# EavnJeong/IEF-VAD

Measured on AMD Instinct MI355X. Metric: snippets/sec at [B,T=256,d=768], higher is better.
Workload: dtype f32 emulated: exact 3-term bf16 split of both fp32 operands, 6 bf16 MFMA products, fp32 accumulate

## Files before the change

### ief-vad_amd/csrc/gemm_bf16.h

```cpp
#pragma once
#include "common.h"
#include "gemm_f32.h"

typedef __bf16 bf16_t;
typedef __bf16 bf16x8 __attribute__((ext_vector_type(8)));
typedef __bf16 bf16x4 __attribute__((ext_vector_type(4)));

struct GemmBProblem {
    const bf16_t* A;
    const bf16_t* W;
    const float* bias;
    float* C;
    bf16_t* Cb;
    const float* R;
    float* C2;
    const float* amaxA;
    const float* amaxW;
    float* amaxC;
};

struct GemmBArgs {
    GemmBProblem p[2];
    int M, N, K;
    int lda, ldc;
// ... 130 lines not shown
#pragma unroll
    for (int a = 0; a < 2; ++a) {
#pragma unroll
        for (int b = 0; b < 2; ++b)
#pragma unroll
            for (int r = 0; r < 16; ++r)
                E[((r & 3) + 8 * (r >> 2) + 4 * h) * GEMMB_EPI_LD + b * 32 + i] = acc[a][b][r];
#pragma unroll
        for (int u = 0; u < 8; ++u) {
            const int lr = rq + 4 * u;
            f32x4 v = *(const f32x4*)(E + lr * GEMMB_EPI_LD + 4 * cq);
            v = v + bv;
            if (epi == EPI_QKV) v = v * scale;
            else if (epi == EPI_BIAS_RELU) {
#pragma unroll
                for (int e = 0; e < 4; ++e) v[e] = (v[e] < 0.f) ? 0.f : v[e];
            } else if (epi == EPI_BIAS_RESID) v = v + res[a * 8 + u];
            else if (epi == EPI_REFINE) v = res[a * 8 + u] - alpha * v;
            const size_t o = (size_t)(mrow + a * 32 + 4 * u) * ldc + nn;
            if (Cb32) *(f32x4*)(Cb32 + o) = v;
            if (Cb16) {
                bf16x4 w;
#pragma unroll
                for (int e = 0; e < 4; ++e) w[e] = (bf16_t)v[e];
                *(bf16x4*)(Cb16 + o) = w;
            }
        }
    }
}


#define GB2_BARRIER()                       \
    do {                                    \
        asm volatile("" ::: "memory");      \
        __builtin_amdgcn_s_barrier();       \
        asm volatile("" ::: "memory");      \
    } while (0)
#define GB2_BM 128
#define GB2_BN 256
#define GB2_BK 32
#define GB2_SLOT ((GB2_BM + GB2_BN) * 16)
#define GB2_STAGES 3
#define GB2_EPI_LD 132
#define GB2_LDS_BYTES (GB2_STAGES * GB2_SLOT * 4)

#ifndef GB2_NT_STORES
#define GB2_NT_STORES 1
#endif
#if GB2_NT_STORES
#define GB2_STORE(ptr, val) __builtin_nontemporal_store((val), (ptr))
#else
#define GB2_STORE(ptr, val) (*(ptr) = (val))
#endif
template <bool MF16, int PASSES>
__device__ __forceinline__ void gemm_wave_epilogue(const GemmBArgs& args, const GemmBProblem& P, float* smem, int m0, int n0,
                                                   int wrow0, int wcol0, f32x16 (&acc)[PASSES][4],
                                                   f32x4 (&acc16)[2 * PASSES][8], float cscale = 1.0f, float* amax_out = nullptr) {
    const int lane = threadIdx.x & 63, wave = threadIdx.x >> 6;
    const int i = lane & 31, h = lane >> 5;
    const int r16 = lane & 15, q16 = lane >> 4;
    const int epi = args.epi, ldc = args.ldc;
    const float alpha = args.alpha;
    const int rq = lane >> 5, cq = lane & 31;
    const int ncol = n0 + wcol0 + 4 * cq;
    const bool has_resid = (epi == EPI_BIAS_RESID || epi == EPI_REFINE || epi == EPI_GATE);
    float* E = smem + wave * (32 * GB2_EPI_LD);
    const f32x4 bv = *(const f32x4*)(P.bias + ncol);
    float* C32 = P.C;
    bf16_t* C16 = P.Cb;
    int nn = ncol;
    f32x4 scale = {1.f, 1.f, 1.f, 1.f};
    if (epi == EPI_HEADS && ncol >= ldc) { C32 = P.C2; nn = ncol - ldc; }
    if (epi == EPI_QKV && ncol < args.qcols) scale = f32x4{alpha, alpha, alpha, alpha};
    float vmax = 0.f;
    const bool wide16 = C16 && !C32 && !has_resid && !amax_out && (epi == EPI_BIAS || epi == EPI_QKV || epi == EPI_BIAS_RELU);
    if (wide16) {
        const int rq4 = lane >> 4, c8 = lane & 15;
        const int ncol8 = n0 + wcol0 + 8 * c8;
        const f32x4 b0 = *(const f32x4*)(P.bias + ncol8), b1 = *(const f32x4*)(P.bias + ncol8 + 4);
        const float sc = (epi == EPI_QKV && ncol8 < args.qcols) ? alpha : 1.f;
#pragma unroll
        for (int a = 0; a < PASSES; ++a) {
            if constexpr (MF16) {
#pragma unroll
                for (int x = 0; x < 2; ++x)
#pragma unroll
                    for (int b = 0; b < 8; ++b)
#pragma unroll
                        for (int r = 0; r < 4; ++r)
                            E[(x * 16 + 4 * q16 + r) * GB2_EPI_LD + b * 16 + r16] = acc16[2 * a + x][b][r];
            } else {
#pragma unroll
                for (int b = 0; b < 4; ++b)
#pragma unroll
                    for (int r = 0; r < 16; ++r)
                        E[((r & 3) + 8 * (r >> 2) + 4 * h) * GB2_EPI_LD + b * 32 + i] = acc[a][b][r];
            }
#pragma unroll
            for (int u = 0; u < 8; ++u) {
                const int row = rq4 + 4 * u;
                f32x4 v0 = *(const f32x4*)(E + row * GB2_EPI_LD + 8 * c8);
                f32x4 v1 = *(const f32x4*)(E + row * GB2_EPI_LD + 8 * c8 + 4);
                v0 = v0 * cscale + b0;
                v1 = v1 * cscale + b1;
                if (epi == EPI_QKV) { v0 = v0 * sc; v1 = v1 * sc; }
                bf16x8 w;
#pragma unroll
                for (int e = 0; e < 4; ++e) {
                    float x0 = v0[e], x1 = v1[e];
                    if (epi == EPI_BIAS_RELU) { x0 = x0 < 0.f ? 0.f : x0; x1 = x1 < 0.f ? 0.f : x1; }
                    w[e] = (bf16_t)x0;
                    w[4 + e] = (bf16_t)x1;
                }
                GB2_STORE((bf16x8*)(C16 + (size_t)(m0 + wrow0 + a * 32 + row) * ldc + ncol8), w);
            }
        }
        return;
    }
#pragma unroll
    for (int a = 0; a < PASSES; ++a) {
        const int mrow = m0 + wrow0 + a * 32 + rq;
        f32x4 res[16];
        if (has_resid) {
#pragma unroll
            for (int u = 0; u < 16; ++u)
                res[u] = *(const f32x4*)(P.R + (size_t)(mrow + 2 * u) * ldc + ncol);
        }
        if constexpr (MF16) {
#pragma unroll
            for (int x = 0; x < 2; ++x)
#pragma unroll
                for (int b = 0; b < 8; ++b)
#pragma unroll
                    for (int r = 0; r < 4; ++r)
                        E[(x * 16 + 4 * q16 + r) * GB2_EPI_LD + b * 16 + r16] = acc16[2 * a + x][b][r];
        } else {
#pragma unroll
            for (int b = 0; b < 4; ++b)
#pragma unroll
                for (int r = 0; r < 16; ++r)
                    E[((r & 3) + 8 * (r >> 2) + 4 * h) * GB2_EPI_LD + b * 32 + i] = acc[a][b][r];
        }
#pragma unroll
        for (int u = 0; u < 16; ++u) {
            f32x4 v = *(const f32x4*)(E + (rq + 2 * u) * GB2_EPI_LD + 4 * cq);
            v = v * cscale + bv;
            if (epi == EPI_QKV) v = v * scale;
            else if (epi == EPI_BIAS_RELU) {
#pragma unroll
                for (int e = 0; e < 4; ++e) v[e] = (v[e] < 0.f) ? 0.f : v[e];
            } else if (epi == EPI_BIAS_RESID) v = v + res[u];
            else if (epi == EPI_REFINE) v = res[u] - alpha * v;
            else if (epi == EPI_GATE) {
#pragma unroll
                for (int e = 0; e < 4; ++e) v[e] = res[u][e] > 0.f ? alpha * v[e] : 0.f;
            }
            const size_t o = (size_t)(mrow + 2 * u) * ldc + nn;
            if (C32) GB2_STORE((f32x4*)(C32 + o), v);
            if (C16) {
                bf16x4 w;
#pragma unroll
                for (int e = 0; e < 4; ++e) w[e] = (bf16_t)v[e];
                GB2_STORE((bf16x4*)(C16 + o), w);
            }
            if (amax_out) {
#pragma unroll
                for (int e = 0; e < 4; ++e) vmax = amax_fold(vmax, v[e]);
            }
        }
    }
// ... 263 lines not shown
```

### ief-vad_amd/csrc/gemm_f32.h

```cpp
#pragma once
#include "common.h"

enum GemmEpilogue {
    EPI_BIAS = 0,
    EPI_QKV = 1,
    EPI_BIAS_RELU = 2,
    EPI_BIAS_RESID = 3,
    EPI_REFINE = 4,
    EPI_HEADS = 5,
    EPI_GATE = 6,
};

struct GemmProblem {
    const float* A;
    const float* W;
    const float* bias;
    float* C;
    const float* R;
    float* C2;
};

struct GemmArgs {
    GemmProblem p[2];
    int M, N, K;
    int lda, ldc;
    int epi;
    float alpha;
    int qcols;
};

#define GEMM_BM 128
#define GEMM_BN 128
#define GEMM_BK 32


template <int TM, int TN>
__device__ __forceinline__ void gemm_prefetch_residual(const GemmArgs& args, const GemmProblem& P, f32x16 (&res)[TM][TN],
                                                       int m0, int n0, int wr, int wc, int i, int h) {
    const int epi = args.epi, ldc = args.ldc;
    if (epi == EPI_BIAS_RESID || epi == EPI_REFINE) {
#pragma unroll
        for (int b = 0; b < TN; ++b)
#pragma unroll
            for (int a = 0; a < TM; ++a)
#pragma unroll
                for (int r = 0; r < 16; ++r)
                    res[a][b][r] = P.R[(size_t)(m0 + wr * 32 * TM + a * 32 + 4 * h + (r & 3) + 8 * (r >> 2)) * ldc +
                                       n0 + wc * 32 * TN + b * 32 + i];
    }
}

template <int TM, int TN>
__device__ __forceinline__ void gemm_epilogue(const GemmArgs& args, const GemmProblem& P, f32x16 (&acc)[TM][TN],
                                              f32x16 (&res)[TM][TN], int m0, int n0, int wr, int wc, int i, int h) {
    const int epi = args.epi, ldc = args.ldc;
    const float alpha = args.alpha;
#pragma unroll
    for (int b = 0; b < TN; ++b) {
        const int n = n0 + wc * 32 * TN + b * 32 + i;
        const float bv = P.bias[n];
        float* Cb = P.C;
        int nn = n;
        float scale = 1.f;
// ... 350 lines not shown
```

### ief-vad_amd/csrc/gemm_split.h

```cpp
#pragma once
#include "gemm_bf16.h"

#ifndef GS_EXP_NODMA
#define GS_EXP_NODMA 0
#endif
#ifndef GS_EXP_NOSPLIT
#define GS_EXP_NOSPLIT 0
#endif
#ifndef GS_EXP_NOBAR
#define GS_EXP_NOBAR 0
#endif
#ifndef GS_PN
#define GS_PN 6
#endif
#define GS_BM 128
#define GS_BK 32
#define GS_A_SLOT (GS_BM * 32)
#define GS_BN_OF(NA) ((NA) == 4 ? 256 : 128)
#define GS_LDS_BYTES_OF(NA) ((2 * GS_A_SLOT + 2 * 3 * GS_BN_OF(NA) * 16) * 4)
#define GS_BN GS_BN_OF(4)
#define GS_LDS_BYTES GS_LDS_BYTES_OF(4)

typedef float f32x2 __attribute__((ext_vector_type(2)));
typedef __bf16 bf16x2 __attribute__((ext_vector_type(2)));
// ... 290 lines not shown
            mfma_row(B, 0, w[1]);                                                                    \
            mfma_row(B, 0, w[0]);                                                                    \
            if (!GS_EXP_NOSPLIT) {                                                                              \
                if (GS_NSPLIT(B) >= 1) split_half(B, v0);                                                       \
                if (GS_NSPLIT(B) == 2) split_half((B) + 1, v1);                                                 \
            }                                                                                                   \
            if ((B) == 7) {                                                                                     \
                _Pragma("unroll") for (int a = 0; a < NA; ++a)                                                  \
                    _Pragma("unroll") for (int p = 0; p < NP; ++p) ap[a][p] = an[a][p];                         \
            }                                                                                                   \
            _Pragma("unroll") for (int d = 0; d < GS_NDMA(B); ++d) dma(GS_NDMA(B) * (B) + d);                   \
            if (GS_NREAD(B) > 0) __builtin_amdgcn_sched_group_barrier(0x100, GS_NREAD(B) > 0 ? GS_NREAD(B) : 1, 0); \
            GS_SLOT(B, 0) GS_SLOT(B, 1) GS_SLOT(B, 2) GS_SLOT(B, 3) GS_SLOT(B, 4) GS_SLOT(B, 5)                 \
            GS_SLOT(B, 6) GS_SLOT(B, 7) GS_SLOT(B, 8) GS_SLOT(B, 9) GS_SLOT(B, 10) GS_SLOT(B, 11)               \
            GS_SLOT(B, 12) GS_SLOT(B, 13) GS_SLOT(B, 14) GS_SLOT(B, 15) GS_SLOT(B, 16) GS_SLOT(B, 17)           \
            GS_SLOT(B, 18) GS_SLOT(B, 19) GS_SLOT(B, 20) GS_SLOT(B, 21) GS_SLOT(B, 22) GS_SLOT(B, 23)           \
            GS_FENCE();                                                                                         \
            if ((B) < 7) {                                                                                      \
                _Pragma("unroll") for (int p = 0; p < NP; ++p) w[p] = wn[p];                                    \
                if (GS_NAREAD(B) >= 1) v0 = vn0;                                                                \
                if (GS_NAREAD(B) == 2) v1 = vn1;                                                                \
            }                                                                                                   \
        }
        GS_STEP(0) GS_STEP(1) GS_STEP(2) GS_STEP(3) GS_STEP(4) GS_STEP(5) GS_STEP(6) GS_STEP(7)
#undef GS_STEP
#undef GS_SLOT
#undef GS_VSLOT
#undef GS_NVALU
#undef GS_NDMA
#undef GS_NREAD
#undef GS_NAREAD
#undef GS_NSPLIT
        GS_DIAG_STAMP(0)
        asm volatile("s_waitcnt vmcnt(0)" ::: "memory");
        asm volatile("s_waitcnt lgkmcnt(0)" ::: "memory");
        GS_DIAG_STAMP(1)
        if (!GS_EXP_NOBAR) GB2_BARRIER();
        GS_DIAG_STAMP(2)
    }
#ifdef GB2_CLOCK_DIAG
    if (threadIdx.x == 0 && P.C2) {
        unsigned long long* dg = (unsigned long long*)P.C2 + 2 * (blockIdx.x + gridDim.x * blockIdx.z);
        dg[0] = __builtin_amdgcn_s_memtime() - dg_c0;
        dg[1] = __builtin_amdgcn_s_memrealtime() - dg_r0;
        unsigned long long* dx = (unsigned long long*)P.C2 + 2 * gridDim.x * gridDim.z + 3 * (blockIdx.x + gridDim.x * blockIdx.z);
        dx[0] = dg_acc[0]; dx[1] = dg_acc[1]; dx[2] = dg_acc[2];
    }
    const unsigned long long dg_loop_end = __builtin_amdgcn_s_memtime();
#endif
#undef GS_PIPE
#undef GS_FENCE
#undef GLDS16
    f32x16 unused[NA / 2][4];
    gemm_wave_epilogue<true, NA / 2>(args, P, smem, m0, n0, wrow0, wcol0, unused, acc16, cscale, F16 ? P.amaxC : nullptr);
#ifdef GB2_CLOCK_DIAG
    if (threadIdx.x == 0 && P.C2) {
        unsigned long long* dy = (unsigned long long*)P.C2 + 5 * gridDim.x * gridDim.z + 2 * (blockIdx.x + gridDim.x * blockIdx.z);
        dy[0] = dg_c0 - dg_entry;
        dy[1] = __builtin_amdgcn_s_memtime() - dg_loop_end;
    }
#endif
}

__global__ __launch_bounds__(256, 1) void iefvad_gemm_split_kernel(GemmBArgs args) {
    extern __shared__ __attribute__((aligned(16))) float smem[];
    gemm_split_body<4>(args, smem);
}

__global__ __launch_bounds__(256, 2) void iefvad_gemm_split_n128_kernel(GemmBArgs args) {
    extern __shared__ __attribute__((aligned(16))) float smem[];
    gemm_split_body<2>(args, smem);
}

__global__ __launch_bounds__(256, 2) void iefvad_gemm_split_f16_n128_kernel(GemmBArgs args) {
    extern __shared__ __attribute__((aligned(16))) float smem[];
    gemm_split_body<2, true>(args, smem);
}

#ifdef GS_EXPERIMENT_F16
__global__ __launch_bounds__(256, 1) void iefvad_gemm_split_f16_kernel(GemmBArgs args) {
    extern __shared__ __attribute__((aligned(16))) float smem[];
    gemm_split_body<4, true>(args, smem);
}
#endif

__global__ __launch_bounds__(256) void iefvad_split_planes_f16_kernel(const float* __restrict__ src, _Float16* __restrict__ planes,
                                                                      size_t n, const float* __restrict__ amax) {
    const float scale = __builtin_ldexpf(1.0f, 13 - amax_exponent(amax_read(amax)));
    const size_t stride = (size_t)gridDim.x * blockDim.x * 4;
    for (size_t i = ((size_t)blockIdx.x * blockDim.x + threadIdx.x) * 4; i < n; i += stride) {
        Split4 s;
        s.r = *(const f32x4*)(src + i) * scale;
#pragma unroll
        for (int p = 0; p < 2; ++p) {
            unsigned d0, d1;
            s.plane_f16(d0, d1, p < 1);
            *(uint2*)(planes + (size_t)p * n + i) = make_uint2(d0, d1);
        }
    }
}
```

### ief-vad_amd/csrc/iefvad.hip

```cpp
#include "../../include/iefvad.h"

#include <hip/hip_runtime.h>
#include <math.h>
#include <stdarg.h>
#include <stdio.h>
#include <stdlib.h>
#include <string.h>

#include <algorithm>
#include <exception>
#include <new>
#include <thread>
#include <vector>

#include "attention_f32.h"
#include "attention_bf16.h"
#include "attention_pbf16.h"
#include "attention_split.h"
#include "common.h"
#include "gather.h"
#include "gemm_f32.h"
#include "gemm_bf16.h"
#include "gemm_split.h"
#include "rowops.h"
// ... 13 lines not shown
static thread_local char g_err[512] = "";

static int fail(const char* fmt, ...) {
    va_list ap;
    va_start(ap, fmt);
    vsnprintf(g_err, sizeof(g_err), fmt, ap);
    va_end(ap);
    return 1;
}

#define HIP_TRY(expr)                                                                            \
    do {                                                                                         \
        hipError_t e_ = (expr);                                                                  \
        if (e_ != hipSuccess) return fail("%s failed: %s (%s:%d)", #expr, hipGetErrorString(e_), \
                                          __FILE__, __LINE__);                                   \
    } while (0)

struct iefvad_handle {
    iefvad_config cfg;
    int D, DH;
    int device;
    bool weights_set;
    bool no_heads_fusion, no_ln_fusion;
    char* iproj_stream[2][IEFVAD_MAX_LAYERS];
    char* heads_stream;
    int chain_min_blocks;
    int rowblock_min_wgs;
    bool no_inproj_chain;
    char* oproj_stream[2][IEFVAD_MAX_LAYERS];
    bool dense_encoder;
    bool persist;
    bool train_attn_unfused;
    bool hostpipe_trace;
    bool no_chain;
    char* chain_stream;
    float* arena;
    size_t arena_floats;
    float* in_w[2][IEFVAD_MAX_LAYERS];
    float* in_b[2][IEFVAD_MAX_LAYERS];
    float* out_w[2][IEFVAD_MAX_LAYERS];
    float* out_b[2][IEFVAD_MAX_LAYERS];
    float* norm_w[2][IEFVAD_MAX_LAYERS];
    float* norm_b[2][IEFVAD_MAX_LAYERS];
    float* whiten_w[2];
    float* whiten_b[2];
    float* head_w[2];
    float* head_b[2];
    float* ref_w1[IEFVAD_MAX_STEPS];
    float* ref_b1[IEFVAD_MAX_STEPS];
    float* ref_w2[IEFVAD_MAX_STEPS];
    float* ref_b2[IEFVAD_MAX_STEPS];
    float* cls_w;
    float* cls_b;
    bf16_t* arena_b;
    bf16_t* in_wb[2][IEFVAD_MAX_LAYERS];
    bf16_t* out_wb[2][IEFVAD_MAX_LAYERS];
    bf16_t* head_wb[2];
    bf16_t* ref_w1b[IEFVAD_MAX_STEPS];
    bf16_t* ref_w2b[IEFVAD_MAX_STEPS];
    bf16_t* arena_s;
    bf16_t* in_ws[2][IEFVAD_MAX_LAYERS];
    bf16_t* out_ws[2][IEFVAD_MAX_LAYERS];
    bf16_t* head_ws[2];
    bf16_t* ref_w1s[IEFVAD_MAX_STEPS];
    bf16_t* ref_w2s[IEFVAD_MAX_STEPS];
    _Float16* arena_h;
    float* amax_dev;
    _Float16* in_wh[2][IEFVAD_MAX_LAYERS];  const float* in_wa[2][IEFVAD_MAX_LAYERS];
    _Float16* out_wh[2][IEFVAD_MAX_LAYERS]; const float* out_wa[2][IEFVAD_MAX_LAYERS];
    _Float16* head_wh[2];                   const float* head_wa[2];
    _Float16* ref_w1h[IEFVAD_MAX_STEPS];    const float* ref_w1a[IEFVAD_MAX_STEPS];
    _Float16* ref_w2h[IEFVAD_MAX_STEPS];    const float* ref_w2a[IEFVAD_MAX_STEPS];
    struct EventPool* events;
    struct GraphCache* graphs;
    struct MetaRing* meta;
    int num_cus;
    bf16_t* arena_st; float* zero_bias; bool tplanes_valid;
    bf16_t* in_wst[2][IEFVAD_MAX_LAYERS]; bf16_t* out_wst[2][IEFVAD_MAX_LAYERS]; bf16_t* head_wst[2];
    bf16_t* ref_w1st[IEFVAD_MAX_STEPS]; bf16_t* ref_w2st[IEFVAD_MAX_STEPS];
    struct HostPipe* hostpipe;
    struct TrainState* train;
    const float* row_scale[2];
};
static const int kAmaxActBase = 256;
static int amax_act_tensors(int L, int K) { return 2 + 6 * L + 2 * K + 1; }
static size_t amax_words(int L, int K, int mb_chunks) {
    return (size_t)kAmaxActBase * IEF_AMAX_FLOATS + (size_t)amax_act_tensors(L, K) * mb_chunks * IEF_AMAX_PARTS;
}

static const int kDefaultMicroBatchF32 = 256;
static const int kDefaultMicroBatchBF16 = 1024;

static int micro_batch(const iefvad_handle* h) {
    if (h->cfg.micro_batch > 0) return h->cfg.micro_batch < 16384 ? h->cfg.micro_batch : 16384;
    return h->cfg.compute == IEFVAD_COMPUTE_F32 ? kDefaultMicroBatchF32 : kDefaultMicroBatchBF16;
}

extern "C" int iefvad_abi_version(void) { return IEFVAD_ABI_VERSION; }

extern "C" const char* iefvad_last_error(void) { return g_err; }

#define IEF_D512 512

static int create_impl(const char* who, bool allow_512, const iefvad_config* cfg, iefvad_handle** out) {
    if (!cfg || !out) return fail("%s: null argument", who);
    *out = nullptr;
// ... 221 lines not shown
    for (int i = 0; i < count; ++i) {
        if (!src[i] || !planes[i] || rows[i] < 0) return fail("iefvad_split_bf16x3_many: entry %d is null or has negative rows", i);
        if (((uintptr_t)src[i] | (uintptr_t)planes[i]) & 15) return fail("iefvad_split_bf16x3_many: entry %d is not 16-byte aligned", i);
        if (int rc = sm.add(src[i], (bf16_t*)planes[i], n[i], rows[i])) return rc;
    }
    return sm.flush();
}

extern "C" int iefvad_split_bf16x3(const float* src, void* planes, size_t n, void* stream) {
    if (!src || !planes) return fail("iefvad_split_bf16x3: null argument");
    return launch_split_planes(src, (bf16_t*)planes, n, (hipStream_t)stream);
}

#define COPY_MANY_MAX 96
struct CopyManyArgs {
    float* dst[COPY_MANY_MAX];
    const float* src[COPY_MANY_MAX];
    unsigned count[COPY_MANY_MAX];
    int n;
};
__global__ __launch_bounds__(256) void iefvad_copy_many_kernel(CopyManyArgs a) {
    float* d = a.dst[blockIdx.y];
    const float* s = a.src[blockIdx.y];
    const unsigned n = a.count[blockIdx.y];
    const unsigned tid = blockIdx.x * 256 + threadIdx.x, nth = gridDim.x * 256;
    if ((((uintptr_t)d | (uintptr_t)s) & 15) == 0) {
        const unsigned n4 = n >> 2;
        for (unsigned i = tid; i < n4; i += nth) ((f32x4*)d)[i] = ((const f32x4*)s)[i];
        for (unsigned i = (n4 << 2) + tid; i < n; i += nth) d[i] = s[i];
    } else {
        for (unsigned i = tid; i < n; i += nth) d[i] = s[i];
    }
}

extern "C" int iefvad_set_weights(iefvad_handle* h, const iefvad_weights* w, void* stream_) {
    if (!h || !w) return fail("iefvad_set_weights: null argument");
    hipStream_t stream = (hipStream_t)stream_;
    const int L = h->cfg.num_layers, K = h->cfg.num_steps;
    const size_t D = h->D, DD = D * D;
    for (int m = 0; m < 2; ++m) {
        for (int l = 0; l < L; ++l)
            if (!w->in_proj_w[m][l] || !w->in_proj_b[m][l] || !w->out_proj_w[m][l] || !w->out_proj_b[m][l] ||
                !w->norm_w[m][l] || !w->norm_b[m][l])
                return fail("iefvad_set_weights: null encoder weight (modality %d layer %d)", m, l);
        if (!w->whiten_w[m] || !w->whiten_b[m] || !w->mu_w[m] || !w->mu_b[m] || !w->logvar_w[m] || !w->logvar_b[m])
            return fail("iefvad_set_weights: null head weight (modality %d)", m);
    }
    for (int k = 0; k < K; ++k)
        if (!w->ref_w1[k] || !w->ref_b1[k] || !w->ref_w2[k] || !w->ref_b2[k])
            return fail("iefvad_set_weights: null refinement weight (step %d)", k);
    if (!w->cls_w || !w->cls_b) return fail("iefvad_set_weights: null classifier weight");

    const size_t total = 2 * L * (3 * DD + 3 * D + DD + D + 2 * D) + 2 * (2 * D) + 2 * (2 * DD + 2 * D) +
                         (size_t)K * (2 * DD + 2 * D) + D + 4;
    if (!h->arena) {
        HIP_TRY(hipSetDevice(h->device));
        HIP_TRY(hipMalloc((void**)&h->arena, total * sizeof(float)));
        h->arena_floats = total;
    }
    float* p = h->arena;
    CopyManyArgs cm;
    cm.n = 0;
    auto flush = [&]() -> hipError_t {
        if (cm.n == 0) return hipSuccess;
        hipLaunchKernelGGL(iefvad_copy_many_kernel, dim3(32, cm.n), dim3(256), 0, stream, cm);
        cm.n = 0;
        return hipGetLastError();
    };
    auto put = [&](float** dst, const float* src, size_t n) -> hipError_t {
        *dst = p;
        p += n;
        cm.dst[cm.n] = *dst; cm.src[cm.n] = src; cm.count[cm.n] = (unsigned)n;
        if (++cm.n == COPY_MANY_MAX) return flush();
        return hipSuccess;
    };
    for (int m = 0; m < 2; ++m) {
        for (int l = 0; l < L; ++l) {
            HIP_TRY(put(&h->in_w[m][l], w->in_proj_w[m][l], 3 * DD));
            HIP_TRY(put(&h->in_b[m][l], w->in_proj_b[m][l], 3 * D));
            HIP_TRY(put(&h->out_w[m][l], w->out_proj_w[m][l], DD));
            HIP_TRY(put(&h->out_b[m][l], w->out_proj_b[m][l], D));
            HIP_TRY(put(&h->norm_w[m][l], w->norm_w[m][l], D));
            HIP_TRY(put(&h->norm_b[m][l], w->norm_b[m][l], D));
        }
        HIP_TRY(put(&h->whiten_w[m], w->whiten_w[m], D));
        HIP_TRY(put(&h->whiten_b[m], w->whiten_b[m], D));
        HIP_TRY(put(&h->head_w[m], w->mu_w[m], DD));
        float* dummy;
        HIP_TRY(put(&dummy, w->logvar_w[m], DD));
        HIP_TRY(put(&h->head_b[m], w->mu_b[m], D));
        HIP_TRY(put(&dummy, w->logvar_b[m], D));
    }
    for (int k = 0; k < K; ++k) {
        HIP_TRY(put(&h->ref_w1[k], w->ref_w1[k], DD));
        HIP_TRY(put(&h->ref_b1[k], w->ref_b1[k], D));
        HIP_TRY(put(&h->ref_w2[k], w->ref_w2[k], DD));
        HIP_TRY(put(&h->ref_b2[k], w->ref_b2[k], D));
    }
    HIP_TRY(put(&h->cls_w, w->cls_w, D));
    HIP_TRY(put(&h->cls_b, w->cls_b, 1));
    HIP_TRY(flush());
    if ((size_t)(p - h->arena) > h->arena_floats) return fail("iefvad_set_weights: arena overflow");
    if (h->cfg.compute == IEFVAD_COMPUTE_BF16) {
        const size_t nb = 2 * (size_t)L * (3 * DD + DD) + 2 * (2 * DD) + (size_t)K * 2 * DD;
        if (!h->arena_b) HIP_TRY(hipMalloc((void**)&h->arena_b, nb * sizeof(bf16_t)));
        bf16_t* q = h->arena_b;
        auto conv = [&](bf16_t** dst, const float* src, size_t n) -> int {
            *dst = q;
            q += n;
            return launch_cast<float>(src, nullptr, nullptr, nullptr, *dst, nullptr, n, 1, stream);
        };
        for (int m = 0; m < 2; ++m) {
            for (int l = 0; l < L; ++l) {
                if (int rc = conv(&h->in_wb[m][l], h->in_w[m][l], 3 * DD)) return rc;
                if (int rc = conv(&h->out_wb[m][l], h->out_w[m][l], DD)) return rc;
            }
            if (int rc = conv(&h->head_wb[m], h->head_w[m], 2 * DD)) return rc;
        }
        for (int k = 0; k < K; ++k) {
            if (int rc = conv(&h->ref_w1b[k], h->ref_w1[k], DD)) return rc;
            if (int rc = conv(&h->ref_w2b[k], h->ref_w2[k], DD)) return rc;
        }
        for (int m = 0; m < 2; ++m)
            for (int l = 0; l < L; ++l) {
                if (!h->oproj_stream[m][l]) HIP_TRY(hipMalloc((void**)&h->oproj_stream[m][l], wstream_bytes()));
                hipLaunchKernelGGL(iefvad_wstream_pack_kernel, dim3(256), dim3(256), 0, stream, h->out_wb[m][l], h->oproj_stream[m][l], 1);
                HIP_TRY(hipGetLastError());
                if (!h->iproj_stream[m][l]) HIP_TRY(hipMalloc((void**)&h->iproj_stream[m][l], wstream_bytes(IC_NPASS)));
                hipLaunchKernelGGL(iefvad_wstream_pack_kernel, dim3(512), dim3(256), 0, stream, h->in_wb[m][l], h->iproj_stream[m][l], IC_NPASS);
                HIP_TRY(hipGetLastError());
            }
        if (!h->heads_stream) HIP_TRY(hipMalloc((void**)&h->heads_stream, heads_stream_bytes()));
        hipLaunchKernelGGL(iefvad_heads_pack_kernel, dim3(512), dim3(256), 0, stream, h->head_wb[0], h->head_wb[1], h->heads_stream);
        HIP_TRY(hipGetLastError());
        if (K > 0) {
            if (!h->chain_stream) HIP_TRY(hipMalloc((void**)&h->chain_stream, chain_stream_bytes(K)));
            ChainPackArgs pa;
            memset(&pa, 0, sizeof(pa));
            for (int k = 0; k < K; ++k) {
                pa.W[2 * k] = h->ref_w1b[k]; pa.bias[2 * k] = h->ref_b1[k];
                pa.W[2 * k + 1] = h->ref_w2b[k]; pa.bias[2 * k + 1] = h->ref_b2[k];
            }
            pa.stream = h->chain_stream;
            pa.K = K;
            hipLaunchKernelGGL(iefvad_chain_pack_kernel, dim3(2048), dim3(256), 0, stream, pa);
            HIP_TRY(hipGetLastError());
        }
    }
    if (h->cfg.compute == IEFVAD_COMPUTE_BF16X6) {
        const size_t nb = 2 * (size_t)L * (3 * DD + DD) + 2 * (2 * DD) + (size_t)K * 2 * DD;
        if (!h->arena_s) HIP_TRY(hipMalloc((void**)&h->arena_s, 3 * nb * sizeof(bf16_t)));
        bf16_t* q = h->arena_s;
        SplitMany sm(stream);
        auto split = [&](bf16_t** dst, const float* src, size_t n) -> int {
// ... 140 lines not shown
        for (int m = 0; m < nz; ++m) {
            b.p[m].A = (const bf16_t*)a.p[m].A; b.p[m].W = (const bf16_t*)a.p[m].W;
            b.p[m].bias = a.p[m].bias; b.p[m].C = a.p[m].C; b.p[m].R = a.p[m].R; b.p[m].C2 = a.p[m].C2;
        }
        dim3 grid((a.M / GB2_BM) * (a.N / GB2_BN), 1, nz);
        hipLaunchKernelGGL(iefvad_gemm_f32_t256_kernel, grid, dim3(256), GB2_LDS_BYTES, stream, b);
    } else if (blocks128 < kF32SmallMaxBlocks128) {
        dim3 grid((a.M / GEMS_BM) * (a.N / GEMS_BN), 1, nz);
        hipLaunchKernelGGL(iefvad_gemm_f32_small_kernel, grid, dim3(256), 0, stream, a);
    } else {
        dim3 grid((a.M / GEMM_BM) * (a.N / GEMM_BN), 1, nz);
        hipLaunchKernelGGL(iefvad_gemm_f32_kernel, grid, dim3(256), 0, stream, a);
    }
    tm.end(e);
    tm.gemm_launches += 1;
    HIP_TRY(hipGetLastError());
    return 0;
}

static int launch_gemm_b(const GemmBArgs& a, int nz, hipStream_t stream, Timer& tm, int stage) {
    hipEvent_t e;
    if (a.N % GB2_BN == 0 && a.M % GB2_BM == 0 && a.K % GB2_BK == 0 && a.K >= 2 * GB2_BK) {
        e = tm.begin(stage);
        if (a.M % GB3_BM == 0 && a.epi != EPI_REFINE && (a.M / GB3_BM) * (a.N / GB2_BN) * nz >= 256) {
            dim3 grid((a.M / GB3_BM) * (a.N / GB2_BN), 1, nz);
            hipLaunchKernelGGL(iefvad_gemm_bf16_w256_kernel, grid, dim3(512), GB3_LDS_BYTES, stream, a);
        } else {
            dim3 grid((a.M / GB2_BM) * (a.N / GB2_BN), 1, nz);
            hipLaunchKernelGGL(iefvad_gemm_bf16_pipe_kernel, grid, dim3(256), GB2_LDS_BYTES, stream, a);
        }
    } else {
        if (a.M % GEMM_BM || a.N % GEMM_BN || a.K % GEMMB_BK)
            return fail("gemm(bf16): shape M=%d N=%d K=%d not a multiple of the %dx%dx%d tile", a.M, a.N, a.K, GEMM_BM,
                        GEMM_BN, GEMMB_BK);
        dim3 grid((a.M / GEMM_BM) * (a.N / GEMM_BN), 1, nz);
        e = tm.begin(stage);
        hipLaunchKernelGGL(iefvad_gemm_bf16_v1_kernel, grid, dim3(256), 0, stream, a);
    }
    tm.end(e);
    tm.gemm_launches += 1;
    HIP_TRY(hipGetLastError());
    return 0;
}

static const int kSplitBN = GS_BN_OF(2);
static const int kSplitMinWgs = 72;
static bool split_eligible(int M, int N, int K, int nz) {
    return M % GS_BM == 0 && N % kSplitBN == 0 && K % 64 == 0 && K >= 64 && (M / GS_BM) * (N / kSplitBN) * nz >= kSplitMinWgs;
}

static int launch_gemm_split(const GemmBArgs& a, int nz, hipStream_t stream, Timer& tm, int stage, bool f16 = false) {
    if (a.M % GS_BM || a.N % kSplitBN || a.K % 64 || a.K < 64)
        return fail("gemm(bf16x6): shape M=%d N=%d K=%d not a multiple of the %dx%dx64 tile", a.M, a.N, a.K, GS_BM, kSplitBN);
    dim3 grid((a.M / GS_BM) * (a.N / kSplitBN), 1, nz);
    hipEvent_t e = tm.begin(stage);
    if (f16) hipLaunchKernelGGL(iefvad_gemm_split_f16_n128_kernel, grid, dim3(256), GS_LDS_BYTES_OF(2), stream, a);
    else hipLaunchKernelGGL(iefvad_gemm_split_n128_kernel, grid, dim3(256), GS_LDS_BYTES_OF(2), stream, a);
    tm.end(e);
    tm.gemm_launches += 1;
    HIP_TRY(hipGetLastError());
    return 0;
}

static size_t in_elem_bytes(int in_dtype) { return in_dtype == IEFVAD_IN_F32 ? 4 : 2; }

struct Proj {
    const float* A32[2];
    const bf16_t* A16[2];
    const float* W32[2];
    const bf16_t* W16[2];
    const bf16_t* Ws[2];
    const _Float16* Wh[2];
    const float* amaxW[2];
    const float* amaxA[2];
    float* amaxC[2];
    const float* bias[2];
    float* C[2];
    bf16_t* Cb[2];
    const float* R[2];
    float* C2[2];
    int N, ldc, epi, nz;
    float alpha;
    int qcols;
};

static int launch_proj(const Proj& p, int compute, bool use_split, int D, int rows, hipStream_t stream, Timer& tm, int stage) {
    const bool bf16 = (compute == IEFVAD_COMPUTE_BF16);
    if (use_split) {
        const bool f16 = (compute == IEFVAD_COMPUTE_FP16X3);
        GemmBArgs g;
        memset(&g, 0, sizeof(g));
        g.M = rows; g.N = p.N; g.K = IEF_D; g.lda = IEF_D; g.ldc = p.ldc; g.epi = p.epi; g.alpha = p.alpha; g.qcols = p.qcols;
        g.wplane = p.N * IEF_D * 2;
        for (int m = 0; m < p.nz; ++m) {
            g.p[m].A = (const bf16_t*)p.A32[m];
            g.p[m].W = f16 ? (const bf16_t*)p.Wh[m] : p.Ws[m];
            g.p[m].bias = p.bias[m]; g.p[m].C = p.C[m]; g.p[m].R = p.R[m]; g.p[m].C2 = p.C2[m];
            if (f16) {
                if (!p.amaxA[m] || !p.amaxW[m]) return fail("gemm(fp16x3): missing running-max word");
                g.p[m].amaxA = p.amaxA[m]; g.p[m].amaxW = p.amaxW[m]; g.p[m].amaxC = p.amaxC[m];
            }
        }
        return launch_gemm_split(g, p.nz, stream, tm, stage, f16);
    }
    if (!bf16) {
        GemmArgs g;
        memset(&g, 0, sizeof(g));
        g.M = rows; g.N = p.N; g.K = D; g.lda = D; g.ldc = p.ldc; g.epi = p.epi; g.alpha = p.alpha; g.qcols = p.qcols;
        for (int m = 0; m < p.nz; ++m) {
            g.p[m].A = p.A32[m]; g.p[m].W = p.W32[m]; g.p[m].bias = p.bias[m]; g.p[m].C = p.C[m]; g.p[m].R = p.R[m];
            g.p[m].C2 = p.C2[m];
        }
        return launch_gemm(g, p.nz, stream, tm, stage);
    }
    GemmBArgs g;
    memset(&g, 0, sizeof(g));
    g.M = rows; g.N = p.N; g.K = IEF_D; g.lda = IEF_D; g.ldc = p.ldc; g.epi = p.epi; g.alpha = p.alpha; g.qcols = p.qcols;
    for (int m = 0; m < p.nz; ++m) {
        g.p[m].A = p.A16[m]; g.p[m].W = p.W16[m]; g.p[m].bias = p.bias[m]; g.p[m].C = p.C[m]; g.p[m].Cb = p.Cb[m];
        g.p[m].R = p.R[m]; g.p[m].C2 = p.C2[m];
    }
    return launch_gemm_b(g, p.nz, stream, tm, stage);
}

static int launch_inproj_chain(iefvad_handle* h, int l, const void* const A[2], bool a_fp32, bf16_t* const C[2], int rows, hipStream_t stream, Timer& tm) {
    InProjChainArgs ia;
    memset(&ia, 0, sizeof(ia));
    for (int m = 0; m < 2; ++m) {
        ia.p[m].A = A[m];
        ia.p[m].stream = h->iproj_stream[m][l]; ia.p[m].bias = h->in_b[m][l]; ia.p[m].C = C[m];
    }
    ia.M = rows; ia.alpha = (1.0f / sqrtf((float)IEF_DH)) * 1.4426950408889634f; ia.wave_stride = (unsigned)wstream_wave_stride_bytes(IC_NPASS);
    hipEvent_t e = tm.begin(ST_QKV);
    if (a_fp32) hipLaunchKernelGGL(iefvad_inproj_chain_f32in_kernel, dim3(rows / IC_BM, 2), dim3(512), IC_LDS_BYTES, stream, ia);
    else hipLaunchKernelGGL(iefvad_inproj_chain_bf16_kernel, dim3(rows / IC_BM, 2), dim3(512), IC_LDS_BYTES, stream, ia);
    tm.end(e);
    tm.gemm_launches += 1;
    HIP_TRY(hipGetLastError());
    return 0;
}
// ... 344 lines not shown
            ha.mu[1] = out->event_mu ? mu_e : nullptr;
            ha.lv[1] = out->event_logvar ? lv_e : nullptr;
            ha.n[0] = out->w_i ? out->w_i + row0 * D : nullptr;
            ha.n[1] = out->w_e ? out->w_e + row0 * D : nullptr;
            ha.z = z;
            ha.zb = chain ? nullptr : zb;
            const bool means = wim_out || wem_out;
            ha.nsum_part = means ? ybuf[0] : nullptr;
            if (int rc = launch_heads_chain(h, ha, rows, factor, stream, tm)) return rc;
            hipEvent_t e;
            if (means) {
                e = tm.begin(ST_FUSION);
                hipLaunchKernelGGL(iefvad_rowmean_finish_kernel, dim3((2 * rows + 255) / 256), dim3(256), 0, stream, ha.nsum_part,
                                   wim_out, wem_out, rows, HC_NPART);
                tm.end(e);
                HIP_TRY(hipGetLastError());
            }
        }

        if (!heads_fused) {
            Proj p;
            memset(&p, 0, sizeof(p));
            p.N = 2 * (int)D; p.ldc = (int)D; p.epi = EPI_HEADS; p.nz = 2;
            for (int m = 0; m < 2; ++m) {
                p.A32[m] = xt[m]; p.A16[m] = xtb[m]; p.W32[m] = h->head_w[m]; p.W16[m] = h->head_wb[m]; p.Ws[m] = h->head_ws[m]; p.bias[m] = h->head_b[m];
                p.Wh[m] = h->head_wh[m]; p.amaxW[m] = h->head_wa[m]; p.amaxA[m] = am_x(L - 1, m);
            }
            p.C[0] = mu_i; p.C2[0] = lv_i; p.C[1] = mu_e; p.C2[1] = lv_e;
            if (int rc = launch_proj(p, c.compute, tail_split, (int)D, rows, stream, tm, ST_HEAD)) return rc;
        }

        if (!heads_fused) {
            FusionArgs fa;
            memset(&fa, 0, sizeof(fa));
            fa.mu_i = mu_i; fa.lv_i = lv_i; fa.mu_e = mu_e; fa.lv_e = lv_e;
            fa.n_i = out->w_i ? out->w_i + row0 * D : nullptr;
            fa.n_e = out->w_e ? out->w_e + row0 * D : nullptr;
            fa.z = z;
            fa.zb = (bf && !chain) ? zb : nullptr;
            fa.n_i_mean = wim_out;
            fa.n_e_mean = wem_out;
            fa.nrows = rows; fa.factor = factor; fa.eps = c.epsilon;
            fa.z_amax = am_z(0);
            hipEvent_t e = tm.begin(ST_FUSION);
            if (d512) hipLaunchKernelGGL(iefvad_fusion_kernel<IEF_D512>, dim3((rows + ROW_WAVES - 1) / ROW_WAVES), dim3(256), 0, stream, fa);
            else hipLaunchKernelGGL(iefvad_fusion_kernel<IEF_D>, dim3((rows + ROW_WAVES - 1) / ROW_WAVES), dim3(256), 0, stream, fa);
            tm.end(e);
            HIP_TRY(hipGetLastError());
        }

        if (chain)
            if (int rc = launch_refine_chain(h, z, out->fused ? z : nullptr, logits, rows, stream, tm)) return rc;

        for (int k = 0; k < K && !chain; ++k) {
            Proj p;
            memset(&p, 0, sizeof(p));
            p.N = (int)D; p.ldc = (int)D; p.epi = EPI_BIAS_RELU; p.nz = 1;
            p.A32[0] = z; p.A16[0] = zb; p.W32[0] = h->ref_w1[k]; p.W16[0] = h->ref_w1b[k]; p.Ws[0] = h->ref_w1s[k]; p.bias[0] = h->ref_b1[k];
            p.Wh[0] = h->ref_w1h[k]; p.amaxW[0] = h->ref_w1a[k]; p.amaxA[0] = am_z(k); p.amaxC[0] = am_h(k);
            p.C[0] = bf ? nullptr : hbuf; p.Cb[0] = bf ? hb : nullptr;
            if (int rc = launch_proj(p, c.compute, tail_split, (int)D, rows, stream, tm, ST_REFINE)) return rc;
            memset(&p, 0, sizeof(p));
            p.N = (int)D; p.ldc = (int)D; p.epi = EPI_REFINE; p.alpha = c.lambda_ref; p.nz = 1;
            p.A32[0] = hbuf; p.A16[0] = hb; p.W32[0] = h->ref_w2[k]; p.W16[0] = h->ref_w2b[k]; p.Ws[0] = h->ref_w2s[k]; p.bias[0] = h->ref_b2[k];
            p.Wh[0] = h->ref_w2h[k]; p.amaxW[0] = h->ref_w2a[k]; p.amaxA[0] = am_h(k); p.amaxC[0] = am_z(k + 1);
            p.C[0] = z; p.R[0] = z; p.Cb[0] = (bf && k + 1 < K) ? zb : nullptr;
            if (int rc = launch_proj(p, c.compute, tail_split, (int)D, rows, stream, tm, ST_REFINE)) return rc;
        }

        if (!chain) {
            hipEvent_t e = tm.begin(ST_SCORER);
            if (d512)
                hipLaunchKernelGGL(iefvad_scorer_kernel<IEF_D512>, dim3((rows + ROW_WAVES - 1) / ROW_WAVES), dim3(256), 0, stream, z,
                                   h->cls_w, h->cls_b, logits, rows);
            else
                hipLaunchKernelGGL(iefvad_scorer_kernel<IEF_D>, dim3((rows + ROW_WAVES - 1) / ROW_WAVES), dim3(256), 0, stream, z,
                                   h->cls_w, h->cls_b, logits, rows);
            tm.end(e);
            HIP_TRY(hipGetLastError());
        }

        if (rg) {
            hipEvent_t e = tm.begin(ST_SCORER);
            if (compacted)
                hipLaunchKernelGGL(iefvad_rows_out_kernel, dim3((rg->valid_rows + 255) / 256), dim3(256), 0, stream, logits, wim_out, wem_out,
                                   rg->logits, rg->w_i_mean, rg->w_e_mean, (const RaggedChunk*)nullptr, rg->valid_rows);
            else
                hipLaunchKernelGGL(iefvad_rows_out_kernel, dim3(nb), dim3(256), 0, stream, logits, wim_out, wem_out, rg->logits,
                                   rg->w_i_mean, rg->w_e_mean, rg->d_chunks, rg->valid_rows);
            tm.end(e);
            HIP_TRY(hipGetLastError());
        }
    }
    return 0;
}

static int forward_impl(iefvad_handle* h, const void* img, const void* ev, int32_t in_dtype, int32_t B, void* workspace,
                        size_t workspace_bytes, const iefvad_outputs* out, hipStream_t stream, Timer& tm) {
    if (!h || !img || !ev || !out) return fail("iefvad_forward: null argument");
    if (!h->weights_set) return fail("iefvad_forward: weights not set");
    if (B <= 0) return fail("iefvad_forward: B must be positive (got %d)", B);
    if (in_dtype != IEFVAD_IN_F32 && in_dtype != IEFVAD_IN_F16 && in_dtype != IEFVAD_IN_BF16)
        return fail("iefvad_forward: unknown in_dtype %d", in_dtype);
    if (!workspace || workspace_bytes < iefvad_workspace_bytes(h, B))
        return fail("iefvad_forward: workspace too small (%zu < %zu bytes)", workspace_bytes, iefvad_workspace_bytes(h, B));
    if (((uintptr_t)workspace & 15) || ((uintptr_t)img & 15) || ((uintptr_t)ev & 15))
        return fail("iefvad_forward: buffers must be 16-byte aligned");
    const int mb = micro_batch(h);
    for (int b0 = 0; b0 < B; b0 += mb) {
        const int nb = (B - b0 < mb) ? (B - b0) : mb;
        const size_t row0 = (size_t)b0 * IEF_T;
        const size_t in_off = row0 * (size_t)h->D * in_elem_bytes(in_dtype);
        if (int rc = forward_pass(h, (const char*)img + in_off, (const char*)ev + in_off, in_dtype, nb, row0, workspace, out, nullptr,
                                  stream, tm))
            return rc;
    }
    return 0;
}

static int video_chunks(int n) { return n < IEF_T ? 1 : n / IEF_T + (n % IEF_T ? 1 : 0); }

struct MetaRing {
    static const int kSlots = 4;
// ... 822 lines not shown
```

### ief-vad_amd/csrc/rowops.h

```cpp
#pragma once
#include <hip/hip_fp16.h>
#include <hip/hip_bf16.h>
#include "common.h"

#define ROW_WAVES 4

typedef __bf16 bf16x4_t __attribute__((ext_vector_type(4)));
__device__ __forceinline__ bf16x4_t to_bf16x4(f32x4 v) {
    bf16x4_t w;
#pragma unroll
    for (int e = 0; e < 4; ++e) w[e] = (__bf16)v[e];
    return w;
}

struct LnArgs {
    const float* x[2];
    float* y[2];
    __bf16* yb[2];
    const float* g1[2];
    const float* b1[2];
    const float* g2[2];
    const float* b2[2];
    int nrows;
    float eps;
// ... 132 lines not shown
    if (row >= a.nrows) return;
    const size_t base = (size_t)row * D + 4 * lane;
    float si = 0.f, se = 0.f, zm = 0.f;
#pragma unroll
    for (int j = 0; j < D / 256; ++j) {
        const size_t o = base + 256 * j;
        const f32x4 mi = *(const f32x4*)(a.mu_i + o), li = *(const f32x4*)(a.lv_i + o);
        const f32x4 me = *(const f32x4*)(a.mu_e + o), le = *(const f32x4*)(a.lv_e + o);
        f32x4 ni, ne, z;
#pragma unroll
        for (int e = 0; e < 4; ++e) {
            float nie, nee, ze;
            fuse_elem(mi[e], li[e], me[e], le[e], a.factor, a.eps, nie, nee, ze);
            ni[e] = nie; ne[e] = nee; z[e] = ze;
            si += ni[e];
            se += ne[e];
            zm = amax_fold(zm, z[e]);
        }
        if (a.n_i) *(f32x4*)(a.n_i + o) = ni;
        if (a.n_e) *(f32x4*)(a.n_e + o) = ne;
        *(f32x4*)(a.z + o) = z;
        if (a.zb) *(bf16x4_t*)(a.zb + o) = to_bf16x4(z);
    }
    if (a.z_amax) amax_store_part(a.z_amax, row / IEF_T, row % IEF_T, wave_max(zm), lane);
    if (a.n_i_mean || a.n_e_mean) {
        si = wave_sum(si) * (1.0f / D);
        se = wave_sum(se) * (1.0f / D);
        if (lane == 0) {
            if (a.n_i_mean) a.n_i_mean[row] = si;
            if (a.n_e_mean) a.n_e_mean[row] = se;
        }
    }
}

template <int D>
__global__ __launch_bounds__(256) void iefvad_scorer_kernel(const float* z, const float* w, const float* b,
                                                             float* logits, int nrows) {
    const int lane = threadIdx.x & 63;
    const int row = blockIdx.x * ROW_WAVES + (threadIdx.x >> 6);
    if (row >= nrows) return;
    const float* zp = z + (size_t)row * D + 4 * lane;
    float s = 0.f;
#pragma unroll
    for (int j = 0; j < D / 256; ++j) {
        const f32x4 zv = *(const f32x4*)(zp + 256 * j);
        const f32x4 wv = *(const f32x4*)(w + 4 * lane + 256 * j);
#pragma unroll
        for (int e = 0; e < 4; ++e) s += zv[e] * wv[e];
    }
    s = wave_sum(s);
    if (lane == 0) logits[row] = s + b[0];
}

template <typename T>
__global__ __launch_bounds__(256) void iefvad_cast_kernel(const T* in0, const T* in1, float* out0, float* out1,
                                                          __bf16* ob0, __bf16* ob1, size_t n) {
    const T* in = blockIdx.y ? in1 : in0;
    float* out = blockIdx.y ? out1 : out0;
    __bf16* ob = blockIdx.y ? ob1 : ob0;
    for (size_t idx = (size_t)blockIdx.x * blockDim.x + threadIdx.x; idx * 4 < n; idx += (size_t)gridDim.x * blockDim.x) {
        const size_t o = idx * 4;
        f32x4 v;
#pragma unroll
        for (int e = 0; e < 4; ++e) v[e] = (float)in[o + e];
        if (out) *(f32x4*)(out + o) = v;
        if (ob) *(bf16x4_t*)(ob + o) = to_bf16x4(v);
    }
}

template <typename T, int D>
__global__ __launch_bounds__(256) void iefvad_cast_scaled_kernel(const T* in0, const T* in1, float* out0, float* out1, __bf16* ob0, __bf16* ob1,
                                                                 size_t n, const float* s0, const float* s1) {
    const T* in = blockIdx.y ? in1 : in0;
    float* out = blockIdx.y ? out1 : out0;
    __bf16* ob = blockIdx.y ? ob1 : ob0;
    const float* sc = blockIdx.y ? s1 : s0;
    for (size_t idx = (size_t)blockIdx.x * blockDim.x + threadIdx.x; idx * 4 < n; idx += (size_t)gridDim.x * blockDim.x) {
        const size_t o = idx * 4;
        const float f = sc ? sc[o / D] : 1.0f;
        f32x4 v;
#pragma unroll
        for (int e = 0; e < 4; ++e) {
            v[e] = (float)in[o + e];
            if (f != 1.0f) {
                float prod = v[e] * f;
                asm volatile("" : "+v"(prod));
                v[e] = (float)(T)prod;
            }
        }
        if (out) *(f32x4*)(out + o) = v;
        if (ob) *(bf16x4_t*)(ob + o) = to_bf16x4(v);
    }
}

__global__ __launch_bounds__(256) void iefvad_amax_kernel(const float* in0, const float* in1, float* out0, float* out1, size_t n) {
    const float* in = blockIdx.y ? in1 : in0;
    float* out = blockIdx.y ? out1 : out0;
    float m = 0.f;
    for (size_t idx = (size_t)blockIdx.x * blockDim.x + threadIdx.x; idx * 4 < n; idx += (size_t)gridDim.x * blockDim.x) {
        const f32x4 v = *(const f32x4*)(in + idx * 4);
#pragma unroll
        for (int e = 0; e < 4; ++e) m = amax_fold(m, v[e]);
    }
    amax_publish(out, wave_max(m), threadIdx.x & 63);
}

// ... 16 lines not shown
```

Before: 4.233 million.

## Fold last refine projection and scorer into a dot-product epilogue

Precomputes, at weight-load time, the classifier vector composed with the final refine step's second projection (lambda-scaled) and its bias. The last refine step's first GEMM then emits per-tile partial dot products of its ReLU output with this folded vector. A small scorer kernel combines these partials with z·cls_w, so the final second-projection GEMM can be skipped when the fused output is not requested. This removes one large GEMM plus its output traffic, at the cost of a slightly heavier epilogue and a different rounding order.

```diff
diff --git a/ief-vad_amd/csrc/gemm_bf16.h b/ief-vad_amd/csrc/gemm_bf16.h
--- a/ief-vad_amd/csrc/gemm_bf16.h
+++ b/ief-vad_amd/csrc/gemm_bf16.h
@@ -206,7 +206,7 @@
 #else
 #define GB2_STORE(ptr, val) (*(ptr) = (val))
 #endif
-template <bool MF16, int PASSES>
+template <bool MF16, int PASSES, bool DOT = false>
 __device__ __forceinline__ void gemm_wave_epilogue(const GemmBArgs& args, const GemmBProblem& P, float* smem, int m0, int n0,
                                                    int wrow0, int wcol0, f32x16 (&acc)[PASSES][4],
                                                    f32x4 (&acc16)[2 * PASSES][8], float cscale = 1.0f, float* amax_out = nullptr) {
@@ -270,6 +270,43 @@
             }
         }
         return;
+    }
+    if constexpr (DOT && MF16) {
+        if (epi == EPI_BIAS_RELU_DOT) {
+            const f32x4 dv = *(const f32x4*)(P.R + ncol);
+            float* part = P.C2 + (n0 + wcol0) / 128;
+            const int ntile = args.N / 128;
+#pragma unroll
+            for (int a = 0; a < PASSES; ++a) {
+                const int mrow = m0 + wrow0 + a * 32 + rq;
+#pragma unroll
+                for (int x = 0; x < 2; ++x)
+#pragma unroll
+                    for (int b = 0; b < 8; ++b)
+#pragma unroll
+                        for (int r = 0; r < 4; ++r)
+                            E[(x * 16 + 4 * q16 + r) * GB2_EPI_LD + b * 16 + r16] = acc16[2 * a + x][b][r];
+#pragma unroll
+                for (int u = 0; u < 16; ++u) {
+                    f32x4 v = *(const f32x4*)(E + (rq + 2 * u) * GB2_EPI_LD + 4 * cq);
+                    v = v * cscale + bv;
+#pragma unroll
+                    for (int e = 0; e < 4; ++e) v[e] = (v[e] < 0.f) ? 0.f : v[e];
+                    if (C32) GB2_STORE((f32x4*)(C32 + (size_t)(mrow + 2 * u) * ldc + ncol), v);
+                    float d = v[0] * dv[0];
+                    d += v[1] * dv[1];
+                    d += v[2] * dv[2];
+                    d += v[3] * dv[3];
+                    d += dpp_take<0xB1, 0xF>(d, d);
+                    d += dpp_take<0x4E, 0xF>(d, d);
+                    d += dpp_take<0x141, 0xF>(d, d);
+                    d += dpp_take<0x140, 0xF>(d, d);
+                    d += dpp_take<0x142, 0xA>(0.f, d);
+                    if (cq == 16) part[(size_t)(mrow + 2 * u) * ntile] = d;
+                }
+            }
+            return;
+        }
     }
 #pragma unroll
     for (int a = 0; a < PASSES; ++a) {
diff --git a/ief-vad_amd/csrc/gemm_f32.h b/ief-vad_amd/csrc/gemm_f32.h
--- a/ief-vad_amd/csrc/gemm_f32.h
+++ b/ief-vad_amd/csrc/gemm_f32.h
@@ -9,6 +9,7 @@
     EPI_REFINE = 4,
     EPI_HEADS = 5,
     EPI_GATE = 6,
+    EPI_BIAS_RELU_DOT = 7,
 };
 
 struct GemmProblem {
diff --git a/ief-vad_amd/csrc/gemm_split.h b/ief-vad_amd/csrc/gemm_split.h
--- a/ief-vad_amd/csrc/gemm_split.h
+++ b/ief-vad_amd/csrc/gemm_split.h
@@ -366,7 +366,7 @@
 #undef GS_FENCE
 #undef GLDS16
     f32x16 unused[NA / 2][4];
-    gemm_wave_epilogue<true, NA / 2>(args, P, smem, m0, n0, wrow0, wcol0, unused, acc16, cscale, F16 ? P.amaxC : nullptr);
+    gemm_wave_epilogue<true, NA / 2, !F16>(args, P, smem, m0, n0, wrow0, wcol0, unused, acc16, cscale, F16 ? P.amaxC : nullptr);
 #ifdef GB2_CLOCK_DIAG
     if (threadIdx.x == 0 && P.C2) {
         unsigned long long* dy = (unsigned long long*)P.C2 + 5 * gridDim.x * gridDim.z + 2 * (blockIdx.x + gridDim.x * blockIdx.z);
diff --git a/ief-vad_amd/csrc/iefvad.hip b/ief-vad_amd/csrc/iefvad.hip
--- a/ief-vad_amd/csrc/iefvad.hip
+++ b/ief-vad_amd/csrc/iefvad.hip
@@ -89,6 +89,7 @@
     float* ref_b2[IEFVAD_MAX_STEPS];
     float* cls_w;
     float* cls_b;
+    float* score_fold;
     bf16_t* arena_b;
     bf16_t* in_wb[2][IEFVAD_MAX_LAYERS];
     bf16_t* out_wb[2][IEFVAD_MAX_LAYERS];
@@ -416,7 +417,7 @@
     if (!w->cls_w || !w->cls_b) return fail("iefvad_set_weights: null classifier weight");
 
     const size_t total = 2 * L * (3 * DD + 3 * D + DD + D + 2 * D) + 2 * (2 * D) + 2 * (2 * DD + 2 * D) +
-                         (size_t)K * (2 * DD + 2 * D) + D + 4;
+                         (size_t)K * (2 * DD + 2 * D) + D + 4 + (D + 4);
     if (!h->arena) {
         HIP_TRY(hipSetDevice(h->device));
         HIP_TRY(hipMalloc((void**)&h->arena, total * sizeof(float)));
@@ -464,6 +465,15 @@
     HIP_TRY(put(&h->cls_w, w->cls_w, D));
     HIP_TRY(put(&h->cls_b, w->cls_b, 1));
     HIP_TRY(flush());
+    p += 3;
+    h->score_fold = nullptr;
+    if (h->cfg.compute == IEFVAD_COMPUTE_BF16X6 && K >= 1) {
+        h->score_fold = p;
+        p += D + 4;
+        hipLaunchKernelGGL(iefvad_scorer_fold_weights_kernel, dim3((unsigned)(D / 16 + 1)), dim3(256), 0, stream, h->ref_w2[K - 1],
+                           h->ref_b2[K - 1], h->cls_w, h->cls_b, h->cfg.lambda_ref, h->score_fold, (int)D);
+        HIP_TRY(hipGetLastError());
+    }
     if ((size_t)(p - h->arena) > h->arena_floats) return fail("iefvad_set_weights: arena overflow");
     if (h->cfg.compute == IEFVAD_COMPUTE_BF16) {
         const size_t nb = 2 * (size_t)L * (3 * DD + DD) + 2 * (2 * DD) + (size_t)K * 2 * DD;
@@ -710,6 +720,8 @@
 static int launch_gemm_split(const GemmBArgs& a, int nz, hipStream_t stream, Timer& tm, int stage, bool f16 = false) {
     if (a.M % GS_BM || a.N % kSplitBN || a.K % 64 || a.K < 64)
         return fail("gemm(bf16x6): shape M=%d N=%d K=%d not a multiple of the %dx%dx64 tile", a.M, a.N, a.K, GS_BM, kSplitBN);
+    if (a.epi == EPI_BIAS_RELU_DOT && (f16 || nz != 1 || !a.p[0].R || !a.p[0].C2))
+        return fail("gemm(bf16x6): the dot-product epilogue takes one bf16x6 problem with its vector (R) and its partial sums (C2)");
     dim3 grid((a.M / GS_BM) * (a.N / kSplitBN), 1, nz);
     hipEvent_t e = tm.begin(stage);
     if (f16) hipLaunchKernelGGL(iefvad_gemm_split_f16_n128_kernel, grid, dim3(256), GS_LDS_BYTES_OF(2), stream, a);
@@ -744,6 +756,8 @@
 
 static int launch_proj(const Proj& p, int compute, bool use_split, int D, int rows, hipStream_t stream, Timer& tm, int stage) {
     const bool bf16 = (compute == IEFVAD_COMPUTE_BF16);
+    if (p.epi == EPI_BIAS_RELU_DOT && !(use_split && compute == IEFVAD_COMPUTE_BF16X6))
+        return fail("gemm: the dot-product epilogue exists in the bf16x6 split kernel only");
     if (use_split) {
         const bool f16 = (compute == IEFVAD_COMPUTE_FP16X3);
         GemmBArgs g;
@@ -1194,14 +1208,34 @@
         if (chain)
             if (int rc = launch_refine_chain(h, z, out->fused ? z : nullptr, logits, rows, stream, tm)) return rc;
 
+        const bool fold = tail_split && c.compute == IEFVAD_COMPUTE_BF16X6 && K >= 1;
+        float* const fold_part = ybuf[0];
+        auto launch_scorer_fold = [&]() -> int {
+            hipEvent_t e = tm.begin(ST_SCORER);
+            hipLaunchKernelGGL((iefvad_scorer_fold_kernel<IEF_D, IEF_D / kSplitBN>), dim3((rows + ROW_WAVES - 1) / ROW_WAVES), dim3(256), 0,
+                               stream, z, h->cls_w, fold_part, h->score_fold, logits, rows);
+            tm.end(e);
+            HIP_TRY(hipGetLastError());
+            return 0;
+        };
+
         for (int k = 0; k < K && !chain; ++k) {
+            const bool dot = fold && k == K - 1;
             Proj p;
             memset(&p, 0, sizeof(p));
             p.N = (int)D; p.ldc = (int)D; p.epi = EPI_BIAS_RELU; p.nz = 1;
             p.A32[0] = z; p.A16[0] = zb; p.W32[0] = h->ref_w1[k]; p.W16[0] = h->ref_w1b[k]; p.Ws[0] = h->ref_w1s[k]; p.bias[0] = h->ref_b1[k];
             p.Wh[0] = h->ref_w1h[k]; p.amaxW[0] = h->ref_w1a[k]; p.amaxA[0] = am_z(k); p.amaxC[0] = am_h(k);
             p.C[0] = bf ? nullptr : hbuf; p.Cb[0] = bf ? hb : nullptr;
+            if (dot) {
+                p.epi = EPI_BIAS_RELU_DOT; p.R[0] = h->score_fold; p.C2[0] = fold_part;
+                if (!out->fused) p.C[0] = nullptr;
+            }
             if (int rc = launch_proj(p, c.compute, tail_split, (int)D, rows, stream, tm, ST_REFINE)) return rc;
+            if (dot) {
+                if (int rc = launch_scorer_fold()) return rc;
+                if (!out->fused) break;
+            }
             memset(&p, 0, sizeof(p));
             p.N = (int)D; p.ldc = (int)D; p.epi = EPI_REFINE; p.alpha = c.lambda_ref; p.nz = 1;
             p.A32[0] = hbuf; p.A16[0] = hb; p.W32[0] = h->ref_w2[k]; p.W16[0] = h->ref_w2b[k]; p.Ws[0] = h->ref_w2s[k]; p.bias[0] = h->ref_b2[k];
@@ -1210,7 +1244,7 @@
             if (int rc = launch_proj(p, c.compute, tail_split, (int)D, rows, stream, tm, ST_REFINE)) return rc;
         }
 
-        if (!chain) {
+        if (!chain && !fold) {
             hipEvent_t e = tm.begin(ST_SCORER);
             if (d512)
                 hipLaunchKernelGGL(iefvad_scorer_kernel<IEF_D512>, dim3((rows + ROW_WAVES - 1) / ROW_WAVES), dim3(256), 0, stream, z,
diff --git a/ief-vad_amd/csrc/rowops.h b/ief-vad_amd/csrc/rowops.h
--- a/ief-vad_amd/csrc/rowops.h
+++ b/ief-vad_amd/csrc/rowops.h
@@ -208,6 +208,54 @@
     if (lane == 0) logits[row] = s + b[0];
 }
 
+template <int D, int NPART>
+__global__ __launch_bounds__(256) void iefvad_scorer_fold_kernel(const float* z, const float* w, const float* part, const float* fold,
+                                                                  float* logits, int nrows) {
+    const int lane = threadIdx.x & 63;
+    const int row = blockIdx.x * ROW_WAVES + (threadIdx.x >> 6);
+    if (row >= nrows) return;
+    const float* zp = z + (size_t)row * D + 4 * lane;
+    float s = 0.f;
+#pragma unroll
+    for (int j = 0; j < D / 256; ++j) {
+        const f32x4 zv = *(const f32x4*)(zp + 256 * j);
+        const f32x4 wv = *(const f32x4*)(w + 4 * lane + 256 * j);
+#pragma unroll
+        for (int e = 0; e < 4; ++e) s += zv[e] * wv[e];
+    }
+    s = wave_sum(s);
+    if (lane == 0) {
+        const float* pp = part + (size_t)row * NPART;
+#pragma unroll
+        for (int t = 0; t < NPART; ++t) s += pp[t];
+        logits[row] = s + fold[D];
+    }
+}
+
+#define FOLD_SEGS 16
+__global__ __launch_bounds__(256) void iefvad_scorer_fold_weights_kernel(const float* __restrict__ w2, const float* __restrict__ b2,
+                                                                         const float* __restrict__ c, const float* __restrict__ bc,
+                                                                         float lambda, float* __restrict__ fold, int D) {
+    __shared__ double part[FOLD_SEGS][16];
+    const int seg = threadIdx.x >> 4, jj = threadIdx.x & 15;
+    const int len = D / FOLD_SEGS, n0 = seg * len;
+    const bool is_s0 = (int)blockIdx.x == D / 16;
+    double s = 0.0;
+    if (!is_s0) {
+        const int j = blockIdx.x * 16 + jj;
+        for (int n = n0; n < n0 + len; ++n) s = __builtin_fma((double)c[n], (double)w2[(size_t)n * D + j], s);
+    } else if (jj == 0) {
+        for (int n = n0; n < n0 + len; ++n) s = __builtin_fma((double)c[n], (double)b2[n], s);
+    }
+    part[seg][jj] = s;
+    __syncthreads();
+    if (seg != 0 || (is_s0 && jj != 0)) return;
+    double t = 0.0;
+    for (int g = 0; g < FOLD_SEGS; ++g) t += part[g][jj];
+    if (!is_s0) fold[blockIdx.x * 16 + jj] = (float)(-(double)lambda * t);
+    else fold[D] = (float)((double)bc[0] - (double)lambda * t);
+}
+
 template <typename T>
 __global__ __launch_bounds__(256) void iefvad_cast_kernel(const T* in0, const T* in1, float* out0, float* out1,
                                                           __bf16* ob0, __bf16* ob1, size_t n) {
```

New measurement: 4.337 million, median of 6. 1.02x the previous value.
